# jy0205/Pyramid-Flow

Hardware: NVIDIA H100
Metric: dit_step_latent_tokens_per_sec (higher is better)
Workload: dtype bf16

## Files before the change

pyramid_flow_b200/csrc/pf_attn.cu:

```cuda
#include <algorithm>
#include <vector>

#include "../../include/pf_b200.h"
#include "pf_common.cuh"

namespace pf {

constexpr int ATT_BM = 128;
constexpr int ATT_BN = 128;
constexpr int ATT_HD = 64;
constexpr int ATT_STAGES = 2;
constexpr int ATT_THREADS = 384;
constexpr int ATT_TILE_BYTES = ATT_BN * ATT_HD * 2;
constexpr int ATT_SMEM_BYTES = (1 + 2 * ATT_STAGES) * ATT_TILE_BYTES + 1024;

struct AttnArgs {
  __nv_bfloat16* out;
  long long ldo;
  int batch, heads, seq, q_tiles;
  float scale_log2;
  const int* seg;
  const int* time;
  const int* sched;
  int sched_stride;
  __nv_bfloat16* peer_out[PF_MAX_PEERS];
  int peer_count, peer_chunk_rows, peer_col_begin;
  float* lse;
};

template <bool kLse>
__global__ void __launch_bounds__(ATT_THREADS, 1)
attn_fwd_kernel(const __grid_constant__ CUtensorMap tm_q, const __grid_constant__ CUtensorMap tm_k,
                const __grid_constant__ CUtensorMap tm_v, const AttnArgs a) {
  extern __shared__ uint8_t smem_raw[];
  uint8_t* smem = reinterpret_cast<uint8_t*>((reinterpret_cast<uintptr_t>(smem_raw) + 1023) & ~uintptr_t(1023));
  uint8_t* smem_q = smem;
  uint8_t* smem_k = smem + ATT_TILE_BYTES;
  uint8_t* smem_v = smem_k + ATT_STAGES * ATT_TILE_BYTES;

  __shared__ __align__(8) uint64_t bar_q;
  __shared__ __align__(8) uint64_t k_full[ATT_STAGES], k_empty[ATT_STAGES], v_full[ATT_STAGES], v_empty[ATT_STAGES];

  const int warp = threadIdx.x >> 5;
  const int lane = threadIdx.x & 31;
  const int wgroup = warp >> 2;
  const int qt = a.q_tiles - 1 - static_cast<int>(blockIdx.x);
  const int h = blockIdx.y;
  const int b = blockIdx.z;
  const int bh = b * a.heads + h;
  const int* sched = a.sched + (static_cast<size_t>(b) * a.q_tiles + qt) * a.sched_stride;
  const int n_kv = sched[0];

  if (threadIdx.x == 0) {
    tma_prefetch_desc(&tm_q);
    tma_prefetch_desc(&tm_k);
    tma_prefetch_desc(&tm_v);
    mbar_init(&bar_q, 1);
    for (int i = 0; i < ATT_STAGES; ++i) {
      mbar_init(&k_full[i], 1);
      mbar_init(&k_empty[i], 8);
      mbar_init(&v_full[i], 1);
      mbar_init(&v_empty[i], 8);
    }
    fence_barrier_init();
  }
  __syncthreads();

  if (wgroup == 0) {
    setmaxnreg_dec<40>();
    if (warp == 0 && elect_one()) {
      mbar_arrive_expect_tx(&bar_q, ATT_TILE_BYTES);
      tma_load_3d(smem_q, &tm_q, &bar_q, 0, qt * ATT_BM, bh);
      int st = 0;
      uint32_t ph = 0;
      for (int j = 0; j < n_kv; ++j) {
        const int kt = sched[1 + j] >> 1;
        mbar_wait(&k_empty[st], ph ^ 1);
        mbar_arrive_expect_tx(&k_full[st], ATT_TILE_BYTES);
        tma_load_3d(smem_k + st * ATT_TILE_BYTES, &tm_k, &k_full[st], 0, kt * ATT_BN, bh);
        mbar_wait(&v_empty[st], ph ^ 1);
        mbar_arrive_expect_tx(&v_full[st], ATT_TILE_BYTES);
        tma_load_3d(smem_v + st * ATT_TILE_BYTES, &tm_v, &v_full[st], 0, kt * ATT_BN, bh);
        if (++st == ATT_STAGES) {
          st = 0;
          ph ^= 1;
        }
      }
    }
    return;
  }

  setmaxnreg_inc<232>();
  const int wg = wgroup - 1;
  const int g4 = lane >> 2, t4 = lane & 3;
  const int row0 = wg * 64 + (warp & 3) * 16 + g4;
  const float c = a.scale_log2;
  const int* sg = a.seg + static_cast<size_t>(b) * a.seq;
  const int* tm = a.time + static_cast<size_t>(b) * a.seq;
  int seg_q[2], time_q[2];
#pragma unroll
  for (int r = 0; r < 2; ++r) {
    const int qpos = qt * ATT_BM + row0 + 8 * r;
    const bool q_valid = qpos < a.seq;
    seg_q[r] = q_valid ? sg[qpos] : -0x7fffffff;
    time_q[r] = q_valid ? tm[qpos] : -0x7fffffff;
  }
  float m_run[2] = {-INFINITY, -INFINITY};
  float l_run[2] = {0.f, 0.f};
  float o[32];
#pragma unroll
  for (int i = 0; i < 32; ++i) o[i] = 0.f;

  mbar_wait(&bar_q, 0);
  const uint64_t dq = make_smem_desc_kmajor_sw128(smem_u32(smem_q) + wg * (64 * 128));
  int st = 0;
  uint32_t ph = 0;
  for (int j = 0; j < n_kv; ++j) {
    const int entry = sched[1 + j];
    const int kt = entry >> 1;
    const bool masked = (entry & 1) != 0;

    float s[64];
    mbar_wait(&k_full[st], ph);
    {
      const uint64_t dk = make_smem_desc_kmajor_sw128(smem_u32(smem_k + st * ATT_TILE_BYTES));
      wgmma_fence();
#pragma unroll
      for (int kk = 0; kk < ATT_HD / 16; ++kk) wgmma_ss_n128(s, dq + 2 * kk, dk + 2 * kk, kk != 0 ? 1u : 0u);
      wgmma_commit();
      wgmma_wait<0>();
      wgmma_reg_fence(s);
    }
    if (lane == 0) mbar_arrive(&k_empty[st]);

    if (masked) {
#pragma unroll
      for (int i = 0; i < 16; ++i) {
#pragma unroll
        for (int e = 0; e < 2; ++e) {
          const int kv = kt * ATT_BN + 8 * i + 2 * t4 + e;
          int sk = 0x7fffffff, tk = 0x7fffffff;
          if (kv < a.seq) {
            sk = __ldg(sg + kv);
            tk = __ldg(tm + kv);
          }
          if (!(sk == seg_q[0] && tk <= time_q[0])) s[4 * i + e] = -INFINITY;
          if (!(sk == seg_q[1] && tk <= time_q[1])) s[4 * i + 2 + e] = -INFINITY;
        }
      }
    }

    float alpha[2];
#pragma unroll
    for (int r = 0; r < 2; ++r) {
      float mx = -INFINITY;
#pragma unroll
      for (int i = 0; i < 16; ++i) mx = fmaxf(mx, fmaxf(s[4 * i + 2 * r], s[4 * i + 2 * r + 1]));
      mx = fmaxf(mx, __shfl_xor_sync(0xffffffffu, mx, 1));
      mx = fmaxf(mx, __shfl_xor_sync(0xffffffffu, mx, 2));
      const float m_new = fmaxf(m_run[r], mx);
      alpha[r] = (m_new == -INFINITY) ? 1.f : ex2_approx_f((m_run[r] - m_new) * c);
      m_run[r] = m_new;
      const float m_ref = (m_new == -INFINITY) ? 0.f : m_new * c;
      float sum = 0.f;
#pragma unroll
      for (int i = 0; i < 16; ++i) {
        const float p0 = ex2_approx_f(fmaf(s[4 * i + 2 * r], c, -m_ref));
        const float p1 = ex2_approx_f(fmaf(s[4 * i + 2 * r + 1], c, -m_ref));
        s[4 * i + 2 * r] = p0;
        s[4 * i + 2 * r + 1] = p1;
        sum += p0 + p1;
      }
      l_run[r] = l_run[r] * alpha[r] + sum;
    }
#pragma unroll
    for (int i = 0; i < 8; ++i) {
      o[4 * i + 0] *= alpha[0];
      o[4 * i + 1] *= alpha[0];
      o[4 * i + 2] *= alpha[1];
      o[4 * i + 3] *= alpha[1];
    }

    mbar_wait(&v_full[st], ph);
    {
      const uint32_t sv = smem_u32(smem_v + st * ATT_TILE_BYTES);
      uint32_t pa[ATT_BN / 16][4];
#pragma unroll
      for (int kk = 0; kk < ATT_BN / 16; ++kk) {
        pa[kk][0] = pack_bf16x2(s[8 * kk + 0], s[8 * kk + 1]);
        pa[kk][1] = pack_bf16x2(s[8 * kk + 2], s[8 * kk + 3]);
        pa[kk][2] = pack_bf16x2(s[8 * kk + 4], s[8 * kk + 5]);
        pa[kk][3] = pack_bf16x2(s[8 * kk + 6], s[8 * kk + 7]);
      }
      wgmma_reg_fence(o);
      wgmma_fence();
#pragma unroll
      for (int kk = 0; kk < ATT_BN / 16; ++kk) {
        const uint64_t dv = make_smem_desc(sv + kk * 2048, ATT_BN * 128, 1024);
        wgmma_rs_n64_tb(o, pa[kk], dv);
      }
      wgmma_commit();
      wgmma_wait<0>();
      wgmma_reg_fence(o);
    }
    if (lane == 0) mbar_arrive(&v_empty[st]);
    if (++st == ATT_STAGES) {
      st = 0;
      ph ^= 1;
    }
  }

#pragma unroll
  for (int r = 0; r < 2; ++r) {
    float l = l_run[r];
    l += __shfl_xor_sync(0xffffffffu, l, 1);
    l += __shfl_xor_sync(0xffffffffu, l, 2);
    const float inv = (l > 0.f) ? 1.f / l : 0.f;
    const int qpos = qt * ATT_BM + row0 + 8 * r;
    if (qpos >= a.seq) continue;
    if constexpr (kLse) {
      if (t4 == 0) a.lse[static_cast<size_t>(bh) * a.seq + qpos] = (l > 0.f) ? (m_run[r] * c + log2f(l)) * 0.6931471805599453f : INFINITY;
    }
    __nv_bfloat16* dst;
    if (a.peer_count > 1) {
      const int pr = qpos / a.peer_chunk_rows;
      dst = a.peer_out[pr] + static_cast<size_t>(qpos - pr * a.peer_chunk_rows) * a.ldo + a.peer_col_begin + h * ATT_HD;
    } else {
      dst = a.out + (static_cast<size_t>(b) * a.seq + qpos) * a.ldo + h * ATT_HD;
    }
#pragma unroll
    for (int i = 0; i < 8; ++i)
      *reinterpret_cast<uint32_t*>(dst + 8 * i + 2 * t4) = pack_bf16x2(o[4 * i + 2 * r] * inv, o[4 * i + 2 * r + 1] * inv);
  }
}

int warmup_attn_bwd();

int warmup_attn() {
  int rc = ensure_dyn_smem(reinterpret_cast<const void*>(attn_fwd_kernel<false>), ATT_SMEM_BYTES, "attn_fwd_kernel");
  if (!rc) rc = ensure_dyn_smem(reinterpret_cast<const void*>(attn_fwd_kernel<true>), ATT_SMEM_BYTES, "attn_fwd_kernel<lse>");
  if (!rc) rc = warmup_attn_bwd();
  return rc;
}

}

extern "C" int pf_attn_build_schedule(const int32_t* seg, const int32_t* time, int32_t batch, int32_t seq,
                                      int32_t* out, int64_t* allowed_pairs) {
  using namespace pf;
  PF_REQUIRE(batch > 0 && seq > 0, "pf_attn_build_schedule: bad shape");
  const int tiles = (seq + 127) / 128;
  const int stride = 1 + tiles;
  if (out == nullptr) return stride;
  PF_REQUIRE(seg && time, "pf_attn_build_schedule: null ids");
  for (int b = 0; b < batch; ++b) {
    const int32_t* sg = seg + static_cast<size_t>(b) * seq;
    const int32_t* tm = time + static_cast<size_t>(b) * seq;
    std::vector<int32_t> tmin(tiles), tmax(tiles), smin(tiles), smax(tiles);
    for (int t = 0; t < tiles; ++t) {
      const int lo = t * 128, hi = std::min(seq, lo + 128);
      int32_t a = tm[lo], bq = tm[lo], c = sg[lo], d = sg[lo];
      for (int i = lo; i < hi; ++i) {
        a = std::min(a, tm[i]);
        bq = std::max(bq, tm[i]);
        c = std::min(c, sg[i]);
        d = std::max(d, sg[i]);
      }
      tmin[t] = a; tmax[t] = bq; smin[t] = c; smax[t] = d;
    }
    int64_t pairs = 0;
    for (int qt = 0; qt < tiles; ++qt) {
      int32_t* row = out + (static_cast<size_t>(b) * tiles + qt) * stride;
      int cnt = 0;
      const int qlo = qt * 128, qhi = std::min(seq, qlo + 128);
      for (int kt = 0; kt < tiles; ++kt) {
        const int klo = kt * 128, khi = std::min(seq, klo + 128);
        if (tmax[qt] < tmin[kt]) continue;
        if (smax[qt] < smin[kt] || smax[kt] < smin[qt]) continue;
        const bool uniform = (smin[qt] == smax[qt]) && (smin[kt] == smax[kt]) && (smin[qt] == smin[kt]);
        const bool full = uniform && (tmin[qt] >= tmax[kt]) && (khi - klo == 128);
        int64_t n_allowed = 0;
        if (full) {
          n_allowed = static_cast<int64_t>(qhi - qlo) * (khi - klo);
        } else {
          for (int i = qlo; i < qhi; ++i)
            for (int j = klo; j < khi; ++j) n_allowed += (sg[i] == sg[j] && tm[i] >= tm[j]) ? 1 : 0;
          if (n_allowed == 0) continue;
        }
        pairs += n_allowed;
        row[1 + cnt] = (kt << 1) | (full ? 0 : 1);
        ++cnt;
      }
      row[0] = cnt;
      for (int i = 1 + cnt; i < stride; ++i) row[i] = 0;
    }
    if (allowed_pairs) allowed_pairs[b] = pairs;
  }
  return stride;
}

extern "C" int pf_attn_fwd_masked(const pf_attn_desc* d, void* stream_) {
  using namespace pf;
  cudaStream_t stream = static_cast<cudaStream_t>(stream_);
  PF_REQUIRE(d && d->q && d->k && d->v && (d->out || d->peer_count > 1) && d->seg && d->time && d->tile_sched, "pf_attn_fwd_masked: null pointer");
  PF_REQUIRE(d->head_dim == ATT_HD, "pf_attn_fwd_masked: head_dim %d unsupported (64 only)", d->head_dim);
  PF_REQUIRE(d->batch > 0 && d->heads > 0 && d->seq > 0, "pf_attn_fwd_masked: bad shape");
  const int q_tiles = (d->seq + ATT_BM - 1) / ATT_BM;
  PF_REQUIRE(d->sched_stride >= 1 + q_tiles, "pf_attn_fwd_masked: schedule stride %d too small", d->sched_stride);
  PF_REQUIRE(d->q_row_begin >= 0 && d->q_row_begin % ATT_BM == 0 && d->q_row_begin < d->seq,
             "pf_attn_fwd_masked: q_row_begin %d must be a multiple of %d inside the sequence", d->q_row_begin, ATT_BM);
  PF_REQUIRE(d->ldo % 8 == 0 && (reinterpret_cast<uintptr_t>(d->out) & 15) == 0, "pf_attn_fwd_masked: out must be 16-byte aligned");
  PF_REQUIRE(d->variant == 0x10 || d->variant == 0x20 || (d->variant >= 0 && d->variant <= 3), "pf_attn_fwd_masked: bad variant 0x%x", d->variant);
  if (d->variant == 0x20)
    PF_REQUIRE(d->group_sched != nullptr && d->group_mask_index != nullptr && d->group_mask_bits != nullptr,
               "pf_attn_fwd_masked: variant 0x%x needs group_sched, group_mask_index and group_mask_bits", d->variant);
  if (d->variant == 0x10)
    PF_REQUIRE(d->pair_sched != nullptr && d->pair_mask_index != nullptr && d->pair_mask_bits != nullptr,
               "pf_attn_fwd_masked: variant 0x%x needs pair_sched, pair_mask_index and pair_mask_bits", d->variant);
  if (d->peer_count > 1) {
    PF_REQUIRE(d->batch == 1 && d->peer_count <= PF_MAX_PEERS && d->peer_chunk_rows > 0 &&
                   static_cast<long long>(d->peer_chunk_rows) * d->peer_count >= d->seq && d->peer_col_begin % 8 == 0,
               "pf_attn_fwd_masked: bad peer layout (batch %d, count %d, chunk rows %d, seq %d)", d->batch, d->peer_count,
               d->peer_chunk_rows, d->seq);
    for (int i = 0; i < d->peer_count; ++i) PF_REQUIRE(d->peer_out[i] != nullptr, "pf_attn_fwd_masked: peer_out[%d] is null", i);
  }
  if (d->lse != nullptr)
    PF_REQUIRE(d->peer_count <= 1 && d->q_row_begin == 0,
               "pf_attn_fwd_masked: lse is computed for whole local launches only (peer_count %d, q_row_begin %d)", d->peer_count,
               d->q_row_begin);
  CUtensorMap tm[3];
  const void* ptrs[3] = {d->q, d->k, d->v};
  for (int i = 0; i < 3; ++i) {
    const uint64_t dims[3] = {ATT_HD, static_cast<uint64_t>(d->seq), static_cast<uint64_t>(d->batch) * d->heads};
    const uint64_t strides[2] = {ATT_HD * 2, static_cast<uint64_t>(d->seq) * ATT_HD * 2};
    const uint32_t box[3] = {ATT_HD, ATT_BN, 1};
    int rc = encode_tensor_map(&tm[i], CU_TENSOR_MAP_DATA_TYPE_BFLOAT16, 3, ptrs[i], dims, strides, box,
                               CU_TENSOR_MAP_SWIZZLE_128B);
    if (rc) return rc;
  }
  AttnArgs a{};
  a.out = static_cast<__nv_bfloat16*>(d->out);
  a.ldo = d->ldo;
  a.batch = d->batch;
  a.heads = d->heads;
  a.seq = d->seq;
  a.q_tiles = q_tiles;
  a.scale_log2 = d->scale * 1.4426950408889634f;
  a.seg = d->seg;
  a.time = d->time;
  a.sched = d->tile_sched;
  a.sched_stride = d->sched_stride;
  a.peer_count = d->peer_count;
  a.peer_chunk_rows = d->peer_chunk_rows;
  a.peer_col_begin = d->peer_col_begin;
  for (int i = 0; i < PF_MAX_PEERS; ++i) a.peer_out[i] = static_cast<__nv_bfloat16*>(d->peer_out[i]);
  a.lse = d->lse;

  if (int rc = warmup_attn()) return rc;
  dim3 grid(q_tiles - d->q_row_begin / ATT_BM, d->heads, d->batch);
  if (a.lse != nullptr)
    attn_fwd_kernel<true><<<grid, ATT_THREADS, ATT_SMEM_BYTES, stream>>>(tm[0], tm[1], tm[2], a);
  else
    attn_fwd_kernel<false><<<grid, ATT_THREADS, ATT_SMEM_BYTES, stream>>>(tm[0], tm[1], tm[2], a);
  return check_launch("pf_attn_fwd_masked");
}
```

pyramid_flow_b200/csrc/pf_common.cuh:

```cuda
#pragma once

#include <cuda.h>
#include <cuda_bf16.h>
#include <cuda_runtime.h>
#include <stdint.h>

namespace pf {

void set_error(const char* fmt, ...);
int  check_launch(const char* what);

#define PF_REQUIRE(cond, ...)                  \
  do {                                         \
    if (!(cond)) {                             \
      ::pf::set_error(__VA_ARGS__);            \
      return -1;                               \
    }                                          \
  } while (0)

int encode_tensor_map(CUtensorMap* map, CUtensorMapDataType dtype, uint32_t rank, const void* base,
                      const uint64_t* dims, const uint64_t* strides_bytes , const uint32_t* box,
                      CUtensorMapSwizzle swizzle,
                      const uint32_t* elem_strides = nullptr );

int num_sms();
int get_option(int key);
int ensure_dyn_smem(const void* kernel, int bytes, const char* what);

__device__ __forceinline__ uint32_t smem_u32(const void* p) {
  return static_cast<uint32_t>(__cvta_generic_to_shared(p));
}

__device__ __forceinline__ bool elect_one() {
  uint32_t pred = 0;
  asm volatile(
      "{\n\t"
      ".reg .b32 %%rx;\n\t"
      ".reg .pred %%px;\n\t"
      "elect.sync %%rx|%%px, 0xffffffff;\n\t"
      "selp.b32 %0, 1, 0, %%px;\n\t"
      "}\n"
      : "=r"(pred));
  return pred != 0;
}

__device__ __forceinline__ void mbar_init(uint64_t* bar, uint32_t count) {
  asm volatile("mbarrier.init.shared::cta.b64 [%0], %1;" ::"r"(smem_u32(bar)), "r"(count) : "memory");
}
__device__ __forceinline__ void fence_barrier_init() {
  asm volatile("fence.mbarrier_init.release.cluster;" ::: "memory");
}
__device__ __forceinline__ void mbar_arrive_expect_tx(uint64_t* bar, uint32_t bytes) {
  asm volatile("mbarrier.arrive.expect_tx.shared::cta.b64 _, [%0], %1;" ::"r"(smem_u32(bar)), "r"(bytes)
               : "memory");
}
__device__ __forceinline__ void mbar_arrive(uint64_t* bar) {
  asm volatile("mbarrier.arrive.shared::cta.b64 _, [%0];" ::"r"(smem_u32(bar)) : "memory");
}
__device__ __forceinline__ bool mbar_try_wait(uint64_t* bar, uint32_t parity) {
  uint32_t ok;
  asm volatile(
      "{\n\t"
      ".reg .pred p;\n\t"
      "mbarrier.try_wait.parity.shared::cta.b64 p, [%1], %2, %3;\n\t"
      "selp.b32 %0, 1, 0, p;\n\t"
      "}\n"
      : "=r"(ok)
      : "r"(smem_u32(bar)), "r"(parity), "r"(0x989680u)
      : "memory");
  return ok != 0;
}
__device__ __forceinline__ bool mbar_test(uint64_t* bar, uint32_t parity) {
  uint32_t ok;
  asm volatile(
      "{\n\t"
      ".reg .pred p;\n\t"
      "mbarrier.test_wait.parity.shared::cta.b64 p, [%1], %2;\n\t"
      "selp.b32 %0, 1, 0, p;\n\t"
      "}\n"
      : "=r"(ok)
      : "r"(smem_u32(bar)), "r"(parity)
      : "memory");
  return ok != 0;
}
__device__ __forceinline__ void mbar_wait(uint64_t* bar, uint32_t parity) {
  while (!mbar_try_wait(bar, parity)) {
  }
}

__device__ __forceinline__ void tma_prefetch_desc(const CUtensorMap* m) {
  asm volatile("prefetch.tensormap [%0];" ::"l"(reinterpret_cast<uint64_t>(m)) : "memory");
}
__device__ __forceinline__ void tma_load_2d(void* smem_dst, const CUtensorMap* m, uint64_t* bar, int c0, int c1) {
  asm volatile(
      "cp.async.bulk.tensor.2d.shared::cluster.global.mbarrier::complete_tx::bytes [%0], [%1, {%3, %4}], [%2];"
      ::"r"(smem_u32(smem_dst)), "l"(reinterpret_cast<uint64_t>(m)), "r"(smem_u32(bar)), "r"(c0), "r"(c1)
      : "memory");
}
__device__ __forceinline__ void tma_load_3d(void* smem_dst, const CUtensorMap* m, uint64_t* bar, int c0, int c1,
                                            int c2) {
  asm volatile(
      "cp.async.bulk.tensor.3d.shared::cluster.global.mbarrier::complete_tx::bytes [%0], [%1, {%3, %4, %5}], [%2];"
      ::"r"(smem_u32(smem_dst)), "l"(reinterpret_cast<uint64_t>(m)), "r"(smem_u32(bar)), "r"(c0), "r"(c1), "r"(c2)
      : "memory");
}
__device__ __forceinline__ void tma_load_4d(void* smem_dst, const CUtensorMap* m, uint64_t* bar, int c0, int c1,
                                            int c2, int c3) {
  asm volatile(
      "cp.async.bulk.tensor.4d.shared::cluster.global.mbarrier::complete_tx::bytes [%0], [%1, {%3, %4, %5, %6}], "
      "[%2];" ::"r"(smem_u32(smem_dst)),
      "l"(reinterpret_cast<uint64_t>(m)), "r"(smem_u32(bar)), "r"(c0), "r"(c1), "r"(c2), "r"(c3)
      : "memory");
}
__device__ __forceinline__ void tma_load_5d(void* smem_dst, const CUtensorMap* m, uint64_t* bar, int c0, int c1,
                                            int c2, int c3, int c4) {
  asm volatile(
      "cp.async.bulk.tensor.5d.shared::cluster.global.mbarrier::complete_tx::bytes [%0], [%1, {%3, %4, %5, %6, "
      "%7}], [%2];" ::"r"(smem_u32(smem_dst)),
      "l"(reinterpret_cast<uint64_t>(m)), "r"(smem_u32(bar)), "r"(c0), "r"(c1), "r"(c2), "r"(c3), "r"(c4)
      : "memory");
}
__device__ __forceinline__ void fence_proxy_async_smem() {
  asm volatile("fence.proxy.async.shared::cta;" ::: "memory");
}
__device__ __forceinline__ void tma_load_2d_multicast(void* smem_dst, const CUtensorMap* m, uint64_t* bar, int c0, int c1,
                                                      uint16_t cta_mask) {
  asm volatile(
      "cp.async.bulk.tensor.2d.shared::cluster.global.mbarrier::complete_tx::bytes.multicast::cluster [%0], [%1, {%3, %4}], "
      "[%2], %5;" ::"r"(smem_u32(smem_dst)),
      "l"(reinterpret_cast<uint64_t>(m)), "r"(smem_u32(bar)), "r"(c0), "r"(c1), "h"(cta_mask)
      : "memory");
}

__device__ __forceinline__ uint32_t cluster_ctarank() {
  uint32_t r;
  asm volatile("mov.u32 %0, %%cluster_ctarank;" : "=r"(r));
  return r;
}
__device__ __forceinline__ void mbar_arrive_cluster(uint64_t* bar, uint32_t cta) {
  asm volatile(
      "{\n\t"
      ".reg .b32 ra;\n\t"
      "mapa.shared::cluster.u32 ra, %0, %1;\n\t"
      "mbarrier.arrive.shared::cluster.b64 _, [ra];\n\t"
      "}\n" ::"r"(smem_u32(bar)), "r"(cta)
      : "memory");
}
__device__ __forceinline__ void cluster_arrive() { asm volatile("barrier.cluster.arrive.release.aligned;" ::: "memory"); }
__device__ __forceinline__ void cluster_wait() { asm volatile("barrier.cluster.wait.acquire.aligned;" ::: "memory"); }

__device__ __forceinline__ void wgmma_fence() { asm volatile("wgmma.fence.sync.aligned;" ::: "memory"); }
__device__ __forceinline__ void wgmma_commit() { asm volatile("wgmma.commit_group.sync.aligned;" ::: "memory"); }
template <int N>
__device__ __forceinline__ void wgmma_wait() {
  asm volatile("wgmma.wait_group.sync.aligned %0;" ::"n"(N) : "memory");
}
template <int N>
__device__ __forceinline__ void wgmma_reg_fence(float (&d)[N]) {
#pragma unroll
  for (int i = 0; i < N; ++i) asm volatile("" : "+f"(d[i])::"memory");
}
template <int REGS>
__device__ __forceinline__ void setmaxnreg_inc() {
  asm volatile("setmaxnreg.inc.sync.aligned.u32 %0;" ::"n"(REGS));
}
template <int REGS>
__device__ __forceinline__ void setmaxnreg_dec() {
  asm volatile("setmaxnreg.dec.sync.aligned.u32 %0;" ::"n"(REGS));
}
__device__ __forceinline__ void named_bar_sync(int id, int threads) {
  asm volatile("bar.sync %0, %1;" ::"r"(id), "r"(threads) : "memory");
}

__device__ __forceinline__ void wgmma_ss_n128(float (&d)[64], uint64_t desc_a, uint64_t desc_b, uint32_t accumulate) {
  asm volatile(
      "{\n\t"
      ".reg .pred p;\n\t"
      "setp.ne.b32 p, %66, 0;\n\t"
      "wgmma.mma_async.sync.aligned.m64n128k16.f32.bf16.bf16 "
      "{%0, %1, %2, %3, %4, %5, %6, %7, %8, %9, %10, %11, %12, %13, %14, %15, %16, %17, %18, %19, %20, %21, %22, %23, %24, %25, %26, %27, %28, %29, %30, %31, %32, %33, %34, %35, %36, %37, %38, %39, %40, %41, %42, %43, %44, %45, %46, %47, %48, %49, %50, %51, %52, %53, %54, %55, %56, %57, %58, %59, %60, %61, %62, %63}, %64, %65, p, 1, 1, 0, 0;\n\t"
      "}\n"
      : "+f"(d[0]), "+f"(d[1]), "+f"(d[2]), "+f"(d[3]), "+f"(d[4]), "+f"(d[5]), "+f"(d[6]), "+f"(d[7]), "+f"(d[8]), "+f"(d[9]), "+f"(d[10]), "+f"(d[11]), "+f"(d[12]), "+f"(d[13]), "+f"(d[14]), "+f"(d[15]), "+f"(d[16]), "+f"(d[17]), "+f"(d[18]), "+f"(d[19]), "+f"(d[20]), "+f"(d[21]), "+f"(d[22]), "+f"(d[23]), "+f"(d[24]), "+f"(d[25]), "+f"(d[26]), "+f"(d[27]), "+f"(d[28]), "+f"(d[29]), "+f"(d[30]), "+f"(d[31]), "+f"(d[32]), "+f"(d[33]), "+f"(d[34]), "+f"(d[35]), "+f"(d[36]), "+f"(d[37]), "+f"(d[38]), "+f"(d[39]), "+f"(d[40]), "+f"(d[41]), "+f"(d[42]), "+f"(d[43]), "+f"(d[44]), "+f"(d[45]), "+f"(d[46]), "+f"(d[47]), "+f"(d[48]), "+f"(d[49]), "+f"(d[50]), "+f"(d[51]), "+f"(d[52]), "+f"(d[53]), "+f"(d[54]), "+f"(d[55]), "+f"(d[56]), "+f"(d[57]), "+f"(d[58]), "+f"(d[59]), "+f"(d[60]), "+f"(d[61]), "+f"(d[62]), "+f"(d[63])
      : "l"(desc_a), "l"(desc_b), "r"(accumulate)
      : "memory");
}
__device__ __forceinline__ void wgmma_ss_n128_e4m3(float (&d)[64], uint64_t desc_a, uint64_t desc_b, uint32_t accumulate) {
  asm volatile(
      "{\n\t"
      ".reg .pred p;\n\t"
      "setp.ne.b32 p, %66, 0;\n\t"
      "wgmma.mma_async.sync.aligned.m64n128k32.f32.e4m3.e4m3 "
      "{%0, %1, %2, %3, %4, %5, %6, %7, %8, %9, %10, %11, %12, %13, %14, %15, %16, %17, %18, %19, %20, %21, %22, %23, %24, %25, %26, %27, %28, %29, %30, %31, %32, %33, %34, %35, %36, %37, %38, %39, %40, %41, %42, %43, %44, %45, %46, %47, %48, %49, %50, %51, %52, %53, %54, %55, %56, %57, %58, %59, %60, %61, %62, %63}, %64, %65, p, 1, 1;\n\t"
      "}\n"
      : "+f"(d[0]), "+f"(d[1]), "+f"(d[2]), "+f"(d[3]), "+f"(d[4]), "+f"(d[5]), "+f"(d[6]), "+f"(d[7]), "+f"(d[8]), "+f"(d[9]), "+f"(d[10]), "+f"(d[11]), "+f"(d[12]), "+f"(d[13]), "+f"(d[14]), "+f"(d[15]), "+f"(d[16]), "+f"(d[17]), "+f"(d[18]), "+f"(d[19]), "+f"(d[20]), "+f"(d[21]), "+f"(d[22]), "+f"(d[23]), "+f"(d[24]), "+f"(d[25]), "+f"(d[26]), "+f"(d[27]), "+f"(d[28]), "+f"(d[29]), "+f"(d[30]), "+f"(d[31]), "+f"(d[32]), "+f"(d[33]), "+f"(d[34]), "+f"(d[35]), "+f"(d[36]), "+f"(d[37]), "+f"(d[38]), "+f"(d[39]), "+f"(d[40]), "+f"(d[41]), "+f"(d[42]), "+f"(d[43]), "+f"(d[44]), "+f"(d[45]), "+f"(d[46]), "+f"(d[47]), "+f"(d[48]), "+f"(d[49]), "+f"(d[50]), "+f"(d[51]), "+f"(d[52]), "+f"(d[53]), "+f"(d[54]), "+f"(d[55]), "+f"(d[56]), "+f"(d[57]), "+f"(d[58]), "+f"(d[59]), "+f"(d[60]), "+f"(d[61]), "+f"(d[62]), "+f"(d[63])
      : "l"(desc_a), "l"(desc_b), "r"(accumulate)
      : "memory");
}
__device__ __forceinline__ void wgmma_ss_n64(float (&d)[32], uint64_t desc_a, uint64_t desc_b, uint32_t accumulate) {
  asm volatile(
      "{\n\t"
      ".reg .pred p;\n\t"
      "setp.ne.b32 p, %34, 0;\n\t"
      "wgmma.mma_async.sync.aligned.m64n64k16.f32.bf16.bf16 "
      "{%0, %1, %2, %3, %4, %5, %6, %7, %8, %9, %10, %11, %12, %13, %14, %15, %16, %17, %18, %19, %20, %21, %22, %23, %24, %25, %26, %27, %28, %29, %30, %31}, %32, %33, p, 1, 1, 0, 0;\n\t"
      "}\n"
      : "+f"(d[0]), "+f"(d[1]), "+f"(d[2]), "+f"(d[3]), "+f"(d[4]), "+f"(d[5]), "+f"(d[6]), "+f"(d[7]), "+f"(d[8]), "+f"(d[9]), "+f"(d[10]), "+f"(d[11]), "+f"(d[12]), "+f"(d[13]), "+f"(d[14]), "+f"(d[15]), "+f"(d[16]), "+f"(d[17]), "+f"(d[18]), "+f"(d[19]), "+f"(d[20]), "+f"(d[21]), "+f"(d[22]), "+f"(d[23]), "+f"(d[24]), "+f"(d[25]), "+f"(d[26]), "+f"(d[27]), "+f"(d[28]), "+f"(d[29]), "+f"(d[30]), "+f"(d[31])
      : "l"(desc_a), "l"(desc_b), "r"(accumulate)
      : "memory");
}
__device__ __forceinline__ void wgmma_rs_n64_tb(float (&d)[32], const uint32_t (&a)[4], uint64_t desc_b) {
  asm volatile(
      "{\n\t"
      ".reg .pred p;\n\t"
      "setp.ne.b32 p, 1, 0;\n\t"
      "wgmma.mma_async.sync.aligned.m64n64k16.f32.bf16.bf16 "
      "{%0, %1, %2, %3, %4, %5, %6, %7, %8, %9, %10, %11, %12, %13, %14, %15, %16, %17, %18, %19, %20, %21, %22, %23, %24, %25, %26, %27, %28, %29, %30, %31}, {%32, %33, %34, %35}, %36, p, 1, 1, 1;\n\t"
      "}\n"
      : "+f"(d[0]), "+f"(d[1]), "+f"(d[2]), "+f"(d[3]), "+f"(d[4]), "+f"(d[5]), "+f"(d[6]), "+f"(d[7]), "+f"(d[8]), "+f"(d[9]), "+f"(d[10]), "+f"(d[11]), "+f"(d[12]), "+f"(d[13]), "+f"(d[14]), "+f"(d[15]), "+f"(d[16]), "+f"(d[17]), "+f"(d[18]), "+f"(d[19]), "+f"(d[20]), "+f"(d[21]), "+f"(d[22]), "+f"(d[23]), "+f"(d[24]), "+f"(d[25]), "+f"(d[26]), "+f"(d[27]), "+f"(d[28]), "+f"(d[29]), "+f"(d[30]), "+f"(d[31])
      : "r"(a[0]), "r"(a[1]), "r"(a[2]), "r"(a[3]), "l"(desc_b)
      : "memory");
}
template <int BN>
__device__ __forceinline__ void wgmma_ss(float (&d)[BN / 2], uint64_t desc_a, uint64_t desc_b, uint32_t accumulate) {
  static_assert(BN == 128 || BN == 64, "wgmma_ss: tile widths 128 and 64 are instantiated");
  if constexpr (BN == 128) wgmma_ss_n128(d, desc_a, desc_b, accumulate);
  else wgmma_ss_n64(d, desc_a, desc_b, accumulate);
}

__device__ __forceinline__ uint64_t make_smem_desc(uint32_t saddr, uint32_t lbo_bytes, uint32_t sbo_bytes) {
  uint64_t d = 0;
  d |= static_cast<uint64_t>((saddr & 0x3FFFFu) >> 4);
  d |= static_cast<uint64_t>((lbo_bytes >> 4) & 0x3FFFu) << 16;
  d |= static_cast<uint64_t>((sbo_bytes >> 4) & 0x3FFFu) << 32;
  d |= static_cast<uint64_t>(1) << 62;
  return d;
}
__device__ __forceinline__ uint64_t make_smem_desc_kmajor_sw128(uint32_t saddr) {
  return make_smem_desc(saddr, 16, 1024);
}

constexpr int PIPE_THREADS = 384;
constexpr int PIPE_CONSUMER_WARPS = 8;
constexpr int PIPE_BM = 128;
constexpr int PIPE_BK = 64;
template <int BN>
struct PipeCfg {
  static constexpr int A_BYTES = PIPE_BM * PIPE_BK * 2;
  static constexpr int B_BYTES = BN * PIPE_BK * 2;
  static constexpr int STAGE_BYTES = A_BYTES + B_BYTES;
  static constexpr int STAGES = (BN >= 128) ? 4 : 6;
  static constexpr int ACC_PITCH = BN + 8;
  static constexpr int ACC_BYTES = PIPE_BM * ACC_PITCH * 4;
  static constexpr int SMEM_BYTES = STAGES * STAGE_BYTES + ACC_BYTES + 1024;
};

template <int BN>
__device__ __forceinline__ void pipe_consume_tile(float (&acc)[BN / 2], uint8_t* smem, uint64_t* full_bar, uint64_t* empty_bar,
                                                  int num_kb, int wg, int& stage, uint32_t& phase) {
  using Cfg = PipeCfg<BN>;
  const int lane = threadIdx.x & 31;
  int prev = -1;
  for (int kb = 0; kb < num_kb; ++kb) {
    mbar_wait(&full_bar[stage], phase);
    const uint32_t sa = smem_u32(smem + stage * Cfg::STAGE_BYTES);
    const uint64_t da = make_smem_desc_kmajor_sw128(sa + wg * (64 * 128));
    const uint64_t db = make_smem_desc_kmajor_sw128(sa + Cfg::A_BYTES);
    wgmma_reg_fence(acc);
    wgmma_fence();
#pragma unroll
    for (int kk = 0; kk < PIPE_BK / 16; ++kk) wgmma_ss<BN>(acc, da + 2 * kk, db + 2 * kk, (kb | kk) != 0 ? 1u : 0u);
    wgmma_commit();
    wgmma_wait<1>();
    if (prev >= 0 && lane == 0) mbar_arrive(&empty_bar[prev]);
    prev = stage;
    if (++stage == Cfg::STAGES) {
      stage = 0;
      phase ^= 1;
    }
  }
  wgmma_wait<0>();
  wgmma_reg_fence(acc);
  if (prev >= 0 && lane == 0) mbar_arrive(&empty_bar[prev]);
}

template <int BN>
__device__ __forceinline__ void pipe_stage_acc(const float (&acc)[BN / 2], float* acc_tile, int wg) {
  const int w = (threadIdx.x >> 5) & 3, lane = threadIdx.x & 31;
  float* r0 = acc_tile + (wg * 64 + w * 16 + (lane >> 2)) * PipeCfg<BN>::ACC_PITCH + 2 * (lane & 3);
  float* r1 = r0 + 8 * PipeCfg<BN>::ACC_PITCH;
#pragma unroll
  for (int i = 0; i < BN / 8; ++i) {
    *reinterpret_cast<float2*>(r0 + 8 * i) = make_float2(acc[4 * i + 0], acc[4 * i + 1]);
    *reinterpret_cast<float2*>(r1 + 8 * i) = make_float2(acc[4 * i + 2], acc[4 * i + 3]);
  }
}

__device__ __forceinline__ uint32_t pack_bf16x2(float lo, float hi) {
  __nv_bfloat162 v = __floats2bfloat162_rn(lo, hi);
  return *reinterpret_cast<uint32_t*>(&v);
}
__device__ __forceinline__ float rcp_approx_f(float x) {
  float y;
  asm("rcp.approx.ftz.f32 %0, %1;" : "=f"(y) : "f"(x));
  return y;
}
__device__ __forceinline__ float ex2_approx_f(float x) {
  float y;
  asm("ex2.approx.ftz.f32 %0, %1;" : "=f"(y) : "f"(x));
  return y;
}
__device__ __forceinline__ float gelu_tanh_f(float x) {
  const float c0 = -2.0f * 0.7978845608028654f * 1.4426950408889634f;
  const float c1 = c0 * 0.044715f;
  const float x2 = x * x;
  const float nu = x * fmaf(x2, c1, c0);
  return x * rcp_approx_f(1.0f + ex2_approx_f(nu));
}
__device__ __forceinline__ float silu_f(float x) {
  return x * rcp_approx_f(1.0f + ex2_approx_f(-1.4426950408889634f * x));
}

}
```

Measured before the change: 124,100.

## Software-pipeline attention QK and PV wgmma with ping-pong warpgroup scheduling

Restructures the attention main loop so that the QK GEMM for the next KV tile is issued together with the PV GEMM for the current tile, and softmax runs while the PV wgmma is in flight. Named barriers alternate the two consumer warpgroups so their tensor-core issue phases interleave (FA3-style ping-pong). The row-max reduction also becomes a tree. The aim is to hide softmax and exponent latency behind tensor-core work. In exchange it raises register pressure (s, pa and o live at once) and adds barrier ordering that could deadlock or serialize if the arrive and sync counts mismatch.

```diff
diff --git a/pyramid_flow_b200/csrc/pf_attn.cu b/pyramid_flow_b200/csrc/pf_attn.cu
--- a/pyramid_flow_b200/csrc/pf_attn.cu
+++ b/pyramid_flow_b200/csrc/pf_attn.cu
@@ -113,49 +113,51 @@
 
   mbar_wait(&bar_q, 0);
   const uint64_t dq = make_smem_desc_kmajor_sw128(smem_u32(smem_q) + wg * (64 * 128));
-  int st = 0;
-  uint32_t ph = 0;
-  for (int j = 0; j < n_kv; ++j) {
-    const int entry = sched[1 + j];
-    const int kt = entry >> 1;
-    const bool masked = (entry & 1) != 0;
-
-    float s[64];
-    mbar_wait(&k_full[st], ph);
-    {
-      const uint64_t dk = make_smem_desc_kmajor_sw128(smem_u32(smem_k + st * ATT_TILE_BYTES));
-      wgmma_fence();
-#pragma unroll
-      for (int kk = 0; kk < ATT_HD / 16; ++kk) wgmma_ss_n128(s, dq + 2 * kk, dk + 2 * kk, kk != 0 ? 1u : 0u);
-      wgmma_commit();
-      wgmma_wait<0>();
-      wgmma_reg_fence(s);
-    }
-    if (lane == 0) mbar_arrive(&k_empty[st]);
-
-    if (masked) {
-#pragma unroll
-      for (int i = 0; i < 16; ++i) {
-#pragma unroll
-        for (int e = 0; e < 2; ++e) {
-          const int kv = kt * ATT_BN + 8 * i + 2 * t4 + e;
-          int sk = 0x7fffffff, tk = 0x7fffffff;
-          if (kv < a.seq) {
-            sk = __ldg(sg + kv);
-            tk = __ldg(tm + kv);
-          }
-          if (!(sk == seg_q[0] && tk <= time_q[0])) s[4 * i + e] = -INFINITY;
-          if (!(sk == seg_q[1] && tk <= time_q[1])) s[4 * i + 2 + e] = -INFINITY;
+
+  auto issue_qk = [&](float (&s)[64], int stage) {
+    const uint64_t dk = make_smem_desc_kmajor_sw128(smem_u32(smem_k + stage * ATT_TILE_BYTES));
+#pragma unroll
+    for (int kk = 0; kk < ATT_HD / 16; ++kk) wgmma_ss_n128(s, dq + 2 * kk, dk + 2 * kk, kk != 0 ? 1u : 0u);
+    wgmma_commit();
+  };
+  auto issue_pv = [&](const uint32_t (&pa)[ATT_BN / 16][4], int stage) {
+    const uint32_t sv = smem_u32(smem_v + stage * ATT_TILE_BYTES);
+#pragma unroll
+    for (int kk = 0; kk < ATT_BN / 16; ++kk) {
+      const uint64_t dv = make_smem_desc(sv + kk * 2048, ATT_BN * 128, 1024);
+      wgmma_rs_n64_tb(o, pa[kk], dv);
+    }
+    wgmma_commit();
+  };
+  auto mask_tile = [&](float (&s)[64], int kt) {
+#pragma unroll
+    for (int i = 0; i < 16; ++i) {
+#pragma unroll
+      for (int e = 0; e < 2; ++e) {
+        const int kv = kt * ATT_BN + 8 * i + 2 * t4 + e;
+        int sk = 0x7fffffff, tk = 0x7fffffff;
+        if (kv < a.seq) {
+          sk = __ldg(sg + kv);
+          tk = __ldg(tm + kv);
         }
+        if (!(sk == seg_q[0] && tk <= time_q[0])) s[4 * i + e] = -INFINITY;
+        if (!(sk == seg_q[1] && tk <= time_q[1])) s[4 * i + 2 + e] = -INFINITY;
       }
     }
-
-    float alpha[2];
+  };
+  auto softmax = [&](float (&s)[64], float (&alpha)[2]) {
 #pragma unroll
     for (int r = 0; r < 2; ++r) {
-      float mx = -INFINITY;
-#pragma unroll
-      for (int i = 0; i < 16; ++i) mx = fmaxf(mx, fmaxf(s[4 * i + 2 * r], s[4 * i + 2 * r + 1]));
+      float m16[16];
+#pragma unroll
+      for (int i = 0; i < 16; ++i) m16[i] = fmaxf(s[4 * i + 2 * r], s[4 * i + 2 * r + 1]);
+#pragma unroll
+      for (int i = 0; i < 8; ++i) m16[i] = fmaxf(m16[i], m16[i + 8]);
+#pragma unroll
+      for (int i = 0; i < 4; ++i) m16[i] = fmaxf(m16[i], m16[i + 4]);
+#pragma unroll
+      for (int i = 0; i < 2; ++i) m16[i] = fmaxf(m16[i], m16[i + 2]);
+      float mx = fmaxf(m16[0], m16[1]);
       mx = fmaxf(mx, __shfl_xor_sync(0xffffffffu, mx, 1));
       mx = fmaxf(mx, __shfl_xor_sync(0xffffffffu, mx, 2));
       const float m_new = fmaxf(m_run[r], mx);
@@ -173,6 +175,16 @@
       }
       l_run[r] = l_run[r] * alpha[r] + sum;
     }
+  };
+  auto mask_and_softmax = [&](float (&s)[64], int entry, float (&alpha)[2]) {
+    if (entry & 1) {
+      mask_tile(s, entry >> 1);
+      softmax(s, alpha);
+    } else {
+      softmax(s, alpha);
+    }
+  };
+  auto rescale_and_pack = [&](const float (&alpha)[2], const float (&s)[64], uint32_t (&pa)[ATT_BN / 16][4]) {
 #pragma unroll
     for (int i = 0; i < 8; ++i) {
       o[4 * i + 0] *= alpha[0];
@@ -180,34 +192,67 @@
       o[4 * i + 2] *= alpha[1];
       o[4 * i + 3] *= alpha[1];
     }
-
-    mbar_wait(&v_full[st], ph);
-    {
-      const uint32_t sv = smem_u32(smem_v + st * ATT_TILE_BYTES);
-      uint32_t pa[ATT_BN / 16][4];
-#pragma unroll
-      for (int kk = 0; kk < ATT_BN / 16; ++kk) {
-        pa[kk][0] = pack_bf16x2(s[8 * kk + 0], s[8 * kk + 1]);
-        pa[kk][1] = pack_bf16x2(s[8 * kk + 2], s[8 * kk + 3]);
-        pa[kk][2] = pack_bf16x2(s[8 * kk + 4], s[8 * kk + 5]);
-        pa[kk][3] = pack_bf16x2(s[8 * kk + 6], s[8 * kk + 7]);
-      }
+#pragma unroll
+    for (int kk = 0; kk < ATT_BN / 16; ++kk) {
+      pa[kk][0] = pack_bf16x2(s[8 * kk + 0], s[8 * kk + 1]);
+      pa[kk][1] = pack_bf16x2(s[8 * kk + 2], s[8 * kk + 3]);
+      pa[kk][2] = pack_bf16x2(s[8 * kk + 4], s[8 * kk + 5]);
+      pa[kk][3] = pack_bf16x2(s[8 * kk + 6], s[8 * kk + 7]);
+    }
+  };
+
+  const int my_turn = 1 + wg, other_turn = 2 - wg;
+  if (n_kv > 0) {
+    float s[64];
+    uint32_t pa[ATT_BN / 16][4];
+    float alpha[2];
+    if (wg == 1) named_bar_arrive(1, 256);
+
+    mbar_wait(&k_full[0], 0);
+    named_bar_sync(my_turn, 256);
+    wgmma_fence();
+    issue_qk(s, 0);
+    named_bar_arrive(other_turn, 256);
+    wgmma_wait<0>();
+    wgmma_reg_fence(s);
+    if (lane == 0) mbar_arrive(&k_empty[0]);
+    mask_and_softmax(s, sched[1], alpha);
+    rescale_and_pack(alpha, s, pa);
+
+    int st = 0;
+    uint32_t ph = 0;
+    for (int j = 1; j < n_kv; ++j) {
+      const int kst = (st + 1 == ATT_STAGES) ? 0 : st + 1;
+      const uint32_t kph = (kst == 0) ? ph ^ 1 : ph;
+      mbar_wait(&k_full[kst], kph);
+      mbar_wait(&v_full[st], ph);
+      named_bar_sync(my_turn, 256);
       wgmma_reg_fence(o);
       wgmma_fence();
-#pragma unroll
-      for (int kk = 0; kk < ATT_BN / 16; ++kk) {
-        const uint64_t dv = make_smem_desc(sv + kk * 2048, ATT_BN * 128, 1024);
-        wgmma_rs_n64_tb(o, pa[kk], dv);
-      }
-      wgmma_commit();
+      issue_qk(s, kst);
+      issue_pv(pa, st);
+      named_bar_arrive(other_turn, 256);
+      wgmma_wait<1>();
+      wgmma_reg_fence(s);
+      if (lane == 0) mbar_arrive(&k_empty[kst]);
+      mask_and_softmax(s, sched[1 + j], alpha);
       wgmma_wait<0>();
       wgmma_reg_fence(o);
-    }
+      if (lane == 0) mbar_arrive(&v_empty[st]);
+      rescale_and_pack(alpha, s, pa);
+      st = kst;
+      ph = kph;
+    }
+
+    mbar_wait(&v_full[st], ph);
+    named_bar_sync(my_turn, 256);
+    wgmma_reg_fence(o);
+    wgmma_fence();
+    issue_pv(pa, st);
+    if (wg == 0) named_bar_arrive(other_turn, 256);
+    wgmma_wait<0>();
+    wgmma_reg_fence(o);
     if (lane == 0) mbar_arrive(&v_empty[st]);
-    if (++st == ATT_STAGES) {
-      st = 0;
-      ph ^= 1;
-    }
   }
 
 #pragma unroll
diff --git a/pyramid_flow_b200/csrc/pf_common.cuh b/pyramid_flow_b200/csrc/pf_common.cuh
--- a/pyramid_flow_b200/csrc/pf_common.cuh
+++ b/pyramid_flow_b200/csrc/pf_common.cuh
@@ -170,6 +170,9 @@
 }
 __device__ __forceinline__ void named_bar_sync(int id, int threads) {
   asm volatile("bar.sync %0, %1;" ::"r"(id), "r"(threads) : "memory");
+}
+__device__ __forceinline__ void named_bar_arrive(int id, int threads) {
+  asm volatile("bar.arrive %0, %1;" ::"r"(id), "r"(threads) : "memory");
 }
 
 __device__ __forceinline__ void wgmma_ss_n128(float (&d)[64], uint64_t desc_a, uint64_t desc_b, uint32_t accumulate) {
```

After: 128,800, median of 6. +3.8%, better.
